# giuvecchio/PyPBR

Hardware: AMD Instinct MI355X
Metric: Mpixels/s Cook-Torrance eval, 4K maps (higher is better)
Workload: dtype f32

## Files before the change

### __graft_entry__.py

```python
import os
import subprocess
import sys

ROOT = os.path.dirname(os.path.abspath(__file__))
if ROOT not in sys.path:
    sys.path.insert(0, ROOT)


def build() -> None:
    subprocess.check_call(["make", "-s", "-j4", "-C", os.path.join(ROOT, "pypbr_amd", "csrc")])
    subprocess.check_call(["make", "-s", "-C", os.path.join(ROOT, "pypbr_amd", "csrc"), "torch_ops"])
    subprocess.check_call(["make", "-s", "-C", os.path.join(ROOT, "oracle")])
    boxcal_src, boxcal_so = os.path.join(ROOT, "tools", "boxcal.hip"), os.path.join(ROOT, "tools", "libboxcal.so")
    if not os.path.exists(boxcal_so) or os.path.getmtime(boxcal_so) < os.path.getmtime(boxcal_src):
        try:
            subprocess.check_call([os.environ.get("HIPCC", "/opt/rocm/bin/hipcc"), "-O3", "--offload-arch=gfx950", "-shared", "-fPIC", boxcal_src, "-o", boxcal_so])
        except (OSError, subprocess.CalledProcessError) as e:
            print("warning: tools/libboxcal.so (bench-side calibration helper, optional) did not build: %s" % e, file=sys.stderr)
    sys.path.insert(0, os.path.join(ROOT, "tools"))
    import check_isa
    report = check_isa.check()
    print("ISA check ok: %d hand-scheduled kernel instantiations; %s" % (sum(1 for r in report if "<" in r.split("vgpr")[0]), report[-1][:120]))
    import pypbr_amd
    from pypbr_amd import _native
    lib = _native.lib()
    for sym in _native.EXPORTS:
        getattr(lib, sym)
    assert lib.pbr_abi_version() == _native.ABI_VERSION
    from pypbr_amd import torch_ops
    assert torch_ops.available(), "pypbr_amd/_pbr_torch_ops.so did not build or load"
    import torch
    for op in ("cook_torrance", "cook_torrance_backward", "fold_gradient", "srgb_to_linear", "linear_to_srgb",
               "metallic_to_diffuse_specular", "diffuse_specular_to_basecolor_metallic", "colour_backward",
               "metallic_to_diffuse_specular_backward", "diffuse_specular_to_basecolor_metallic_backward", "resize", "resize_backward",
               "normal_from_height", "normal_from_height_backward", "normal_transform", "normal_transform_backward"):
        getattr(torch.ops.pbr_hip, op)
    print("build ok: %s (ABI %d), pypbr_amd %s" % (_native.LIB_PATH, lib.pbr_abi_version(), pypbr_amd.__version__))


def smoke() -> None:
    import torch
    sys.path.insert(0, os.path.join(ROOT, "oracle"))
    import torch_oracle
    from pypbr_amd.materials import BasecolorMetallicMaterial
    from pypbr_amd.models import CookTorranceBRDF

    assert torch.cuda.is_available(), "smoke() needs a ROCm device"
    g = torch.Generator().manual_seed(2024)
    H, W = 96, 128
    albedo = torch.rand(3, H, W, generator=g)
    nxy = torch.rand(2, H, W, generator=g) - 0.5
    normal = torch.cat([nxy, torch.ones(1, H, W)], 0)
    normal = normal / normal.norm(dim=0, keepdim=True)
    rough = torch.rand(1, H, W, generator=g) * 0.85 + 0.15
    metal = torch.rand(1, H, W, generator=g)
    view, light, inten = torch.tensor([0.0, 0.0, 1.0]), torch.tensor([0.1, 0.1, 1.0]), torch.tensor([1.0, 1.0, 1.0])

    mat = BasecolorMetallicMaterial(albedo=albedo, normal=normal, roughness=rough, metallic=metal).to("cuda:0")
    out = CookTorranceBRDF(light_type="point")(mat, view, light, inten, 1.0)
    torch.cuda.synchronize()
    assert out.shape == (3, H, W) and out.device.type == "cuda"
    ref = torch_oracle.cook_torrance(albedo, normal, rough, metal, None, view=view, light=light, intensity=inten,
                                     light_type="point", light_size=1.0)
# ... 10 lines not shown
```

### include/pbr_hip.h

```cpp
#ifndef PBR_HIP_H
#define PBR_HIP_H

#include <stddef.h>
#include <stdint.h>

#ifdef __cplusplus
extern "C" {
#endif

#define PBR_HIP_ABI_VERSION 9
#define PBR_MAX_LIGHTS 16

enum {
    PBR_OK = 0,
    PBR_ERR_NULL_MAP = -1,
    PBR_ERR_WORKFLOW = -2,
    PBR_ERR_LIGHT_TYPE = -3,
    PBR_ERR_SHAPE = -4,
    PBR_ERR_DTYPE = -5,
    PBR_ERR_CHANNELS = -6,
    PBR_ERR_NO_DEVICE = -7,
    PBR_ERR_UNSUPPORTED = -8
};

// ... 48 lines not shown
    int32_t n_lights;
    int32_t albedo_is_srgb;
    int32_t specular_is_srgb;
    int32_t return_srgb;

    pbr_map albedo;
    pbr_map normal;
    pbr_map roughness;
    pbr_map metallic;
    pbr_map specular;
    void *out;

    float view_dir[3];
    float light_size;
    float lights[PBR_MAX_LIGHTS][3];
    float intensities[PBR_MAX_LIGHTS][3];

    int32_t schedule;
    int32_t map_height;
    int32_t map_width;
    int32_t reserved;
    int64_t out_batch_stride;
    int64_t out_channel_stride;
    const void *device_params;
    const pbr_tuning *tuning;
} pbr_render_desc;

#define PBR_SCHEDULE_AUTO 0
#define PBR_SCHEDULE_LINEAR 1
#define PBR_SCHEDULE_XCD(c) (1 + (c))

int pbr_cook_torrance(const pbr_render_desc *desc, void *stream);

int pbr_cook_torrance_autotune(const pbr_render_desc *desc, void *stream, int32_t *schedule);

enum { PBR_BLEND_SIGN_COMPUTE = 0, PBR_BLEND_SIGN_GIVEN = 1 };
typedef struct pbr_blend_desc {
    pbr_map albedo, normal, roughness, metallic, specular;
    pbr_map mask;
    int32_t sign_mode;
    int32_t reserved;
} pbr_blend_desc;
int pbr_blend_normal_sign(const pbr_render_desc *desc, const pbr_blend_desc *blend, void *workspace, void *stream);
int pbr_cook_torrance_blend(const pbr_render_desc *desc, const pbr_blend_desc *blend, void *workspace, void *stream);

int pbr_blend_backward_serves(const pbr_render_desc *desc);
typedef struct pbr_map_grads { void *albedo, *normal, *roughness, *metallic, *specular; } pbr_map_grads;
int pbr_cook_torrance_blend_backward(const pbr_render_desc *desc, const pbr_blend_desc *blend, void *workspace, const void *grad_out,
                                     const pbr_map_grads *g_material1, const pbr_map_grads *g_material2, void *g_mask, void *stream);

int pbr_cook_torrance_backward(const pbr_render_desc *desc, const void *grad_out, void *g_albedo,
                               void *g_normal, void *g_roughness, void *g_metallic, void *g_specular,
                               void *stream);

size_t pbr_backward_folded_workspace_bytes(const pbr_render_desc *desc);
int pbr_cook_torrance_backward_folded(const pbr_render_desc *desc, const void *grad_out, void *g_albedo, void *g_normal,
                                      void *g_roughness, void *g_metallic, void *g_specular, void *workspace, void *stream);

size_t pbr_param_grad_workspace_bytes(const pbr_render_desc *desc);
int pbr_cook_torrance_backward_params(const pbr_render_desc *desc, const void *grad_out, void *g_albedo,
                                      void *g_normal, void *g_roughness, void *g_metallic, void *g_specular,
                                      void *g_params, void *workspace, void *stream);

size_t pbr_mse_step_workspace_bytes(const pbr_render_desc *desc);
int pbr_cook_torrance_mse_step(const pbr_render_desc *desc, const void *target, void *g_albedo, void *g_normal, void *g_roughness,
                               void *g_metallic, void *g_specular, void *loss, void *workspace, void *stream);
// ... 92 lines not shown
```

### pypbr_amd/_native.py

```python
import ctypes
import os

_HERE = os.path.dirname(os.path.abspath(__file__))
LIB_PATH = os.environ.get("PBR_HIP_LIB") or os.path.join(_HERE, "libpbr_hip.so")

ABI_VERSION = 9
RESIZE_TWO_PASS, RESIZE_STRIP, RESIZE_TWO_TAP, RESIZE_BAND_WALK, RESIZE_ROW_WALK = range(5)
MAX_LIGHTS = 16

F32, F16 = 0, 1
LIGHT_DIRECTIONAL, LIGHT_POINT = 0, 1
WORKFLOW_METALLIC, WORKFLOW_SPECULAR, WORKFLOW_CONVERTED = 0, 1, 2
(_TUNE_RESERVED_0, TUNE_BLOCK_LOG2, TUNE_F16_VEC, TUNE_LDS_BYTES, _TUNE_RESERVED_4, TUNE_BATCH_INNER, TUNE_SCALAR_BASE, TUNE_MAX_VEC, TUNE_BWD_RUN,
 TUNE_MSE_STREAM, TUNE_TILE_REPEAT, TUNE_RESIZE_UP2) = range(12)

TUNE_COUNT, TUNE_SLOTS, TUNE_UNSET = 12, 32, -2 ** 31
TUNE_NAMES = {"block_log2": TUNE_BLOCK_LOG2, "f16_vec": TUNE_F16_VEC, "lds_bytes": TUNE_LDS_BYTES, "batch_inner": TUNE_BATCH_INNER, "scalar_base": TUNE_SCALAR_BASE, "max_vec": TUNE_MAX_VEC,
              "bwd_run": TUNE_BWD_RUN, "mse_stream": TUNE_MSE_STREAM, "tile_repeat": TUNE_TILE_REPEAT, "resize_up2": TUNE_RESIZE_UP2}

OK = 0
ERR_NULL_MAP, ERR_WORKFLOW, ERR_LIGHT_TYPE, ERR_SHAPE, ERR_DTYPE, ERR_CHANNELS, ERR_NO_DEVICE = -1, -2, -3, -4, -5, -6, -7
ERR_UNSUPPORTED = -8

EXPORTS = (
    "pbr_cook_torrance", "pbr_srgb_to_linear", "pbr_linear_to_srgb", "pbr_metallic_to_specular",
    "pbr_specular_to_metallic", "pbr_decode_normal", "pbr_abi_version", "pbr_error_string",
    "pbr_kernel_name", "pbr_bytes_per_pixel", "pbr_set_tuning", "pbr_render_desc_size",
    "pbr_resize_workspace_bytes", "pbr_resize_bilinear", "pbr_resize_form", "pbr_cook_torrance_backward",
    "pbr_blend_maps", "pbr_blend_sigmoid_mask", "pbr_blend_gradient_mask", "pbr_cook_torrance_autotune",
    "pbr_cook_torrance_blend", "pbr_fold_gradient", "pbr_decode_normal_backward",
    "pbr_blend_normal_sign", "pbr_blend_backward_serves", "pbr_blend_maps_backward", "pbr_param_grad_workspace_bytes", "pbr_cook_torrance_backward_params",
    "pbr_srgb_to_linear_backward", "pbr_linear_to_srgb_backward", "pbr_metallic_to_specular_backward",
    "pbr_specular_to_metallic_backward", "pbr_resize_backward_workspace_bytes", "pbr_resize_bilinear_backward",
    "pbr_blend_sigmoid_mask_backward", "pbr_cook_torrance_blend_backward", "pbr_fold_gradient_typed",
    "pbr_mse_step_workspace_bytes", "pbr_cook_torrance_mse_step", "pbr_scale_by_device_scalar", "pbr_scale_list_by_device_scalar", "pbr_device_params_bytes", "pbr_prepare_device_params", "pbr_tuning_init", "pbr_build_id", "pbr_unpack_image",
    "pbr_backward_folded_workspace_bytes", "pbr_cook_torrance_backward_folded",
    "pbr_normal_from_height", "pbr_normal_from_height_backward", "pbr_normal_transform", "pbr_normal_transform_backward",
)


class PbrMap(ctypes.Structure):
    _fields_ = [("data", ctypes.c_void_p), ("batch_stride", ctypes.c_int64), ("channel_stride", ctypes.c_int64)]


class Tuning(ctypes.Structure):
    _fields_ = [("knob", ctypes.c_int32 * TUNE_SLOTS)]

    @classmethod
    def of(cls, **knobs):
        t = cls()
        for i in range(TUNE_SLOTS):
            t.knob[i] = TUNE_UNSET
        for name, value in knobs.items():
            t.knob[TUNE_NAMES[name]] = int(value)
        return t


class RenderDesc(ctypes.Structure):
    _fields_ = [
        ("abi_version", ctypes.c_int32), ("batch", ctypes.c_int32), ("height", ctypes.c_int32),
        ("width", ctypes.c_int32), ("height_total", ctypes.c_int32), ("y_offset", ctypes.c_int32),
        ("map_dtype", ctypes.c_int32), ("out_dtype", ctypes.c_int32), ("workflow", ctypes.c_int32),
        ("light_type", ctypes.c_int32), ("n_lights", ctypes.c_int32), ("albedo_is_srgb", ctypes.c_int32),
        ("specular_is_srgb", ctypes.c_int32), ("return_srgb", ctypes.c_int32),
        ("albedo", PbrMap), ("normal", PbrMap), ("roughness", PbrMap), ("metallic", PbrMap), ("specular", PbrMap),
        ("out", ctypes.c_void_p),
        ("view_dir", ctypes.c_float * 3), ("light_size", ctypes.c_float),
        ("lights", (ctypes.c_float * 3) * MAX_LIGHTS), ("intensities", (ctypes.c_float * 3) * MAX_LIGHTS),
        ("schedule", ctypes.c_int32), ("map_height", ctypes.c_int32), ("map_width", ctypes.c_int32),
        ("reserved", ctypes.c_int32),
# ... 16 lines not shown
BLEND_SIGN_COMPUTE, BLEND_SIGN_GIVEN = 0, 1


SCHEDULE_AUTO, SCHEDULE_LINEAR = 0, 1


def schedule_xcd(c: int) -> int:
    return 1 + c


class NativeLibraryError(RuntimeError):
    pass


_lib = None


def lib():
    global _lib
    if _lib is not None:
        return _lib
    import torch
    if not os.path.exists(LIB_PATH):
        raise NativeLibraryError(
            "%s is missing: build it with `python -c 'import __graft_entry__ as g; g.build()'` "
            "or `make -C pypbr_amd/csrc`.  pypbr_amd has no CPU fallback." % LIB_PATH)
    try:
        L = ctypes.CDLL(LIB_PATH)
    except OSError as e:
        raise NativeLibraryError("cannot load %s: %s" % (LIB_PATH, e)) from e
    vp, i32, i64, sz = ctypes.c_void_p, ctypes.c_int32, ctypes.c_int64, ctypes.c_size_t
    L.pbr_cook_torrance.argtypes = [ctypes.POINTER(RenderDesc), vp]
    L.pbr_cook_torrance.restype = ctypes.c_int
    L.pbr_cook_torrance_autotune.argtypes = [ctypes.POINTER(RenderDesc), vp, ctypes.POINTER(ctypes.c_int32)]
    L.pbr_cook_torrance_autotune.restype = ctypes.c_int
    L.pbr_cook_torrance_blend.argtypes = [ctypes.POINTER(RenderDesc), ctypes.POINTER(BlendDesc), vp, vp]
    L.pbr_cook_torrance_blend.restype = ctypes.c_int
    L.pbr_cook_torrance_blend_backward.argtypes = [ctypes.POINTER(RenderDesc), ctypes.POINTER(BlendDesc), vp, vp, ctypes.POINTER(MapGrads),
                                                   ctypes.POINTER(MapGrads), vp, vp]
    L.pbr_cook_torrance_blend_backward.restype = ctypes.c_int
    L.pbr_blend_normal_sign.argtypes = [ctypes.POINTER(RenderDesc), ctypes.POINTER(BlendDesc), vp, vp]
    L.pbr_blend_normal_sign.restype = ctypes.c_int
    L.pbr_blend_backward_serves.argtypes = [ctypes.POINTER(RenderDesc)]
    L.pbr_blend_backward_serves.restype = ctypes.c_int
    L.pbr_param_grad_workspace_bytes.argtypes = [ctypes.POINTER(RenderDesc)]
    L.pbr_param_grad_workspace_bytes.restype = ctypes.c_size_t
    L.pbr_cook_torrance_backward_params.argtypes = [ctypes.POINTER(RenderDesc), vp, vp, vp, vp, vp, vp, vp, vp, vp]
    L.pbr_cook_torrance_backward_params.restype = ctypes.c_int
    L.pbr_fold_gradient.argtypes = [vp, vp, i32, i32, i32, i32, i32, i32, ctypes.c_int, vp]
    L.pbr_fold_gradient.restype = ctypes.c_int
    L.pbr_mse_step_workspace_bytes.argtypes = [ctypes.POINTER(RenderDesc)]
    L.pbr_mse_step_workspace_bytes.restype = ctypes.c_size_t
    L.pbr_cook_torrance_mse_step.argtypes = [ctypes.POINTER(RenderDesc), vp, vp, vp, vp, vp, vp, vp, vp, vp]
    L.pbr_cook_torrance_mse_step.restype = ctypes.c_int
    L.pbr_scale_by_device_scalar.argtypes = [vp, sz, ctypes.c_int, vp, vp]
    L.pbr_scale_by_device_scalar.restype = ctypes.c_int
    L.pbr_scale_list_by_device_scalar.argtypes = [ctypes.POINTER(vp), ctypes.POINTER(sz), ctypes.c_int, ctypes.c_int, vp, vp]
    L.pbr_scale_list_by_device_scalar.restype = ctypes.c_int
    L.pbr_device_params_bytes.argtypes = []
    L.pbr_device_params_bytes.restype = ctypes.c_size_t
    L.pbr_prepare_device_params.argtypes = [ctypes.POINTER(RenderDesc), vp, vp, vp, i32, vp, vp]
    L.pbr_prepare_device_params.restype = ctypes.c_int
    L.pbr_fold_gradient_typed.argtypes = [vp, vp, i32, i32, i32, i32, i32, i32, ctypes.c_int, ctypes.c_int, vp]
    L.pbr_fold_gradient_typed.restype = ctypes.c_int
    L.pbr_cook_torrance_backward.argtypes = [ctypes.POINTER(RenderDesc), vp, vp, vp, vp, vp, vp, vp]
    L.pbr_cook_torrance_backward.restype = ctypes.c_int
# ... 128 lines not shown
```

### pypbr_amd/csrc/cook_torrance.hip

```cpp
#include <hip/hip_runtime.h>

#include <algorithm>

#include "ct_launch.hpp"

namespace pbr {

static constexpr int kKnobRules[PBR_TUNE_COUNT] = {
     1,  0,  8,  -1,  0,  -1,
     1,  8,  -1,  1,  -1,  1};
std::atomic<int> g_knobs[PBR_TUNE_COUNT] = {
    {kKnobRules[0]}, {kKnobRules[1]}, {kKnobRules[2]}, {kKnobRules[3]}, {kKnobRules[4]}, {kKnobRules[5]}, {kKnobRules[6]}, {kKnobRules[7]},
    {kKnobRules[8]}, {kKnobRules[9]}, {kKnobRules[10]}, {kKnobRules[11]}};
thread_local const pbr_tuning *t_tuning = nullptr;

struct KernelEntry { KernelFn fn; const char *name; };

template <int LIGHT, int WF, typename TI, typename TO>
static KernelFn pick_variant(int vec, bool multi) {
    if constexpr (sizeof(TI) == 2) {
        if (vec == 8 && !multi) {
            return cook_torrance_kernel<LIGHT, WF, TI, TO, 8, false, true>;
        }
    }
    if (vec == 1) return multi ? cook_torrance_kernel<LIGHT, WF, TI, TO, 1, true, false>
                               : cook_torrance_kernel<LIGHT, WF, TI, TO, 1, false, false>;
    return multi ? cook_torrance_kernel<LIGHT, WF, TI, TO, 4, true, true> : cook_torrance_kernel<LIGHT, WF, TI, TO, 4, false, true>;
}

template <int LIGHT, int WF>
static KernelFn pick_types(int in_dt, int out_dt, int vec, bool multi) {
    if (in_dt == PBR_F32) return out_dt == PBR_F32 ? pick_variant<LIGHT, WF, float, float>(vec, multi)
                                                   : pick_variant<LIGHT, WF, float, __half>(vec, multi);
    if (out_dt == PBR_F32) return pick_variant<LIGHT, WF, __half, float>(vec, multi);
    return pick_variant<LIGHT, WF, __half, __half>(vec, multi);
}

static KernelEntry pick_kernel(const pbr_render_desc *d, int vec) {
    static thread_local char name[96];
    static const char *const wf_names[3] = {"metallic", "specular", "converted"};
    const bool multi = d->n_lights > 1, point = d->light_type == PBR_LIGHT_POINT;
    const int idt = d->map_dtype, odt = d->out_dtype;
    const int nb = batch_group(d, vec);
    if (repeat_inner(d)) {
        std::snprintf(name, sizeof(name), "ctr_%s_%s_%s_%s_v4%s", point ? "point" : "directional", wf_names[d->workflow],
                      idt == PBR_F32 ? "f32" : "f16", odt == PBR_F32 ? "f32" : "f16", multi ? "_multi" : "");
        return KernelEntry{pick_repeat_kernel(d), name};
    }
    if (nb) {
        std::snprintf(name, sizeof(name), "ctb_%s_%s_%s_%s_v2_b%d", point ? "point" : "directional", wf_names[d->workflow],
                      idt == PBR_F32 ? "f32" : "f16", odt == PBR_F32 ? "f32" : "f16", nb);
        return KernelEntry{pick_batch_kernel(d, nb), name};
    }
    std::snprintf(name, sizeof(name), "ct_%s_%s_%s_%s_v%d%s", point ? "point" : "directional", wf_names[d->workflow],
                  idt == PBR_F32 ? "f32" : "f16", odt == PBR_F32 ? "f32" : "f16", vec, multi ? "_multi" : "");
    return KernelEntry{with_light_workflow(d, [&](auto L, auto W) -> KernelFn { return pick_types<L(), W()>(idt, odt, vec, multi); }), name};
}

}

namespace pbr {
struct HostParams { float view[3]; float lights[PBR_MAX_LIGHTS][3]; float inten[PBR_MAX_LIGHTS][3]; };
__global__ __launch_bounds__(64) void prepare_device_params_kernel(const float *__restrict__ view, const float *__restrict__ lights,
                                                                   const float *__restrict__ inten, int intensity_rows, int n_lights, int light_type,
                                                                   const HostParams hp, DevParams *__restrict__ out) {
    const int i = threadIdx.x;
    float raw[3];
    for (int c = 0; c < 3; ++c) raw[c] = view ? view[c] : hp.view[c];
    float V[3];
    normalize_host(raw, V);
    auto intensity = [&](int l, int c) { return inten ? inten[3 * (intensity_rows == 1 ? 0 : l) + c] : hp.inten[l][c]; };
    if (i == 0) {
        int grey = 1;
        for (int l = 0; l < n_lights; ++l)
            if (intensity(l, 0) != intensity(l, 1) || intensity(l, 0) != intensity(l, 2)) grey = 0;
        for (int c = 0; c < 3; ++c) { out->V[c] = V[c]; out->raw_view[c] = raw[c]; }
        out->grey = grey;
    }
    if (i < n_lights) {
        float L[3], I[3];
        for (int c = 0; c < 3; ++c) { L[c] = lights ? lights[3 * i + c] : hp.lights[i][c]; I[c] = intensity(i, c); }
        LightU u;
        fold_light(light_type, V, L, I, u);
        out->lights[i] = u;
        for (int c = 0; c < 3; ++c) out->raw_lights[i][c] = L[c];
    }
}
}

extern "C" {

int pbr_cook_torrance(const pbr_render_desc *d, void *stream) {
    using namespace pbr;
    const TuningScope tuning(d);
    const int rc = validate(d);
    if (rc != PBR_OK) return rc;
    if (nan_light_size(d)) return fill_result_nan(d, static_cast<hipStream_t>(stream));
    const int vec = pick_vec(d);
    KArgs k;
    if (repeat_inner(d)) {
        fill_repeat_args(d, k);
        if (k.n_tiles < 0) return PBR_ERR_SHAPE;
        const KernelEntry e = pick_kernel(d, 4);
        hipLaunchKernelGGL(e.fn, dim3((unsigned)k.n_tiles, 1, 1), dim3(1u << k.bt_log2, 1, 1), g_lds_bytes >= 0 ? (size_t)g_lds_bytes : 0,
                           static_cast<hipStream_t>(stream), k);
        return launch_status();
    }
    const int nb = batch_group(d, vec);
    if (nb) {
        pbr_render_desc g = *d;
        g.batch = d->batch / nb;
        fill_args(&g, 2, k);
        if (g_scalar_base != 2) k.sbase = 0;
    } else {
        fill_args(d, vec, k);
    }
    if (k.n_tiles < 0) return PBR_ERR_SHAPE;
    const bool tiled = k.tiled != 0;
    const KernelEntry e = pick_kernel(d, vec);
    const bool fp32_one_light = d->map_dtype == PBR_F32 && d->n_lights == 1 && k.bt_log2 == 6 && !tiled;
    size_t lds = g_lds_bytes >= 0 ? (size_t)g_lds_bytes : (fp32_one_light ? kLdsFor11WavesPerCu : 0);
    if (k.xpose) lds = std::max(lds, (size_t)kXposeLdsPerWave << (k.bt_log2 - 6));
    hipLaunchKernelGGL(e.fn, dim3((unsigned)k.n_tiles, 1, 1), dim3(1u << k.bt_log2, 1, 1), lds,
                       static_cast<hipStream_t>(stream), k);
    return launch_status();
}

int pbr_cook_torrance_autotune(const pbr_render_desc *d, void *stream, int32_t *schedule) {
    using namespace pbr;
    const int rc = validate(d);
    if (rc != PBR_OK) return rc;
    if (!schedule) return PBR_ERR_NULL_MAP;
    const int32_t cands[2] = {PBR_SCHEDULE_LINEAR, PBR_SCHEDULE_XCD(6)};
    float best[2] = {3.4e38f, 3.4e38f};
    hipStream_t st = static_cast<hipStream_t>(stream);
    hipEvent_t e0, e1;
    hipError_t created = hipEventCreate(&e0);
    if (created == hipSuccess) created = hipEventCreate(&e1);
    if (created != hipSuccess) return call_status(created);
    pbr_render_desc t = *d;
    int err = PBR_OK;
    const int reps = 4;
    for (int round = 0; round < 3 && err == PBR_OK; ++round) {
        for (int c = 0; c < 2 && err == PBR_OK; ++c) {
            t.schedule = cands[c];
            if ((err = pbr_cook_torrance(&t, stream)) != PBR_OK) break;
            hipError_t he = hipEventRecord(e0, st);
            for (int i = 0; i < reps && err == PBR_OK; ++i) err = pbr_cook_torrance(&t, stream);
            if (he == hipSuccess) he = hipEventRecord(e1, st);
            if (he == hipSuccess) he = hipEventSynchronize(e1);
            float ms = 0.0f;
            if (he == hipSuccess) he = hipEventElapsedTime(&ms, e0, e1);
            if (he != hipSuccess) { err = hip_code(he); break; }
            if (ms < best[c]) best[c] = ms;
        }
    }
    (void)hipEventDestroy(e0); (void)hipEventDestroy(e1);
    if (err != PBR_OK) return err;
    *schedule = best[1] < best[0] ? cands[1] : cands[0];
    return PBR_OK;
}

const char *pbr_kernel_name(const pbr_render_desc *d) {
    const pbr::TuningScope tuning(d);
    if (pbr::validate(d) != PBR_OK) return nullptr;
    return pbr::pick_kernel(d, pbr::pick_vec(d)).name;
}

int pbr_bytes_per_pixel(const pbr_render_desc *d) {
    if (pbr::validate(d) != PBR_OK) return 0;
    const int ein = d->map_dtype == PBR_F32 ? 4 : 2, eout = d->out_dtype == PBR_F32 ? 4 : 2;
    int ch = 3 + 1;
    if (d->normal.data) ch += 3;
    ch += d->workflow == PBR_WORKFLOW_SPECULAR ? 3 : 1;
    if (pbr::is_tiled(d)) {
        const int64_t reps = ((int64_t)d->height_total / d->map_height) * ((int64_t)d->width / d->map_width);
        return (int)((ch * ein + reps - 1) / reps) + 3 * eout;
    }
    return ch * ein + 3 * eout;
}

int pbr_set_tuning(int knob, int value) {
    if (knob < 0 || knob >= PBR_TUNE_COUNT) return -1;
    return pbr::g_knobs[knob].exchange(value == PBR_TUNE_UNSET ? pbr::kKnobRules[knob] : value, std::memory_order_relaxed);
}

void pbr_tuning_init(pbr_tuning *t) {
    if (!t) return;
    for (int i = 0; i < PBR_TUNE_SLOTS; ++i) t->knob[i] = PBR_TUNE_UNSET;
}

size_t pbr_device_params_bytes(void) { return sizeof(pbr::DevParams); }

int pbr_prepare_device_params(const pbr_render_desc *d, const void *view_dir, const void *lights, const void *intensities,
                              int32_t intensity_rows, void *block, void *stream) {
    using namespace pbr;
    if (!d || !block) return PBR_ERR_NULL_MAP;
    if (d->abi_version != PBR_HIP_ABI_VERSION || d->n_lights < 1 || d->n_lights > PBR_MAX_LIGHTS) return PBR_ERR_SHAPE;
    if (d->light_type != PBR_LIGHT_POINT && d->light_type != PBR_LIGHT_DIRECTIONAL) return PBR_ERR_LIGHT_TYPE;
    if (intensities && intensity_rows != 1 && intensity_rows != d->n_lights) return PBR_ERR_SHAPE;
    HostParams hp;
    for (int c = 0; c < 3; ++c) hp.view[c] = d->view_dir[c];
    for (int i = 0; i < PBR_MAX_LIGHTS; ++i)
        for (int c = 0; c < 3; ++c) { hp.lights[i][c] = d->lights[i][c]; hp.inten[i][c] = d->intensities[i][c]; }
    hipLaunchKernelGGL(prepare_device_params_kernel, dim3(1), dim3(64), 0, static_cast<hipStream_t>(stream), static_cast<const float *>(view_dir),
                       static_cast<const float *>(lights), static_cast<const float *>(intensities), (int)intensity_rows, (int)d->n_lights,
                       (int)d->light_type, hp, static_cast<DevParams *>(block));
    return launch_status();
}

}
```

### pypbr_amd/models.py

```python
import collections
import os
import threading
import weakref
from abc import ABC
from typing import Optional

import torch
import torch.nn as nn
from torch import Tensor

from . import _native
from . import functional as F_
from .materials import MaterialBase, _normalised


DEVICE_CACHE_CAP = int(os.environ.get("PBR_DEVICE_CACHE_CAP", str(4 << 30)))
_DEVICE_CACHES = collections.OrderedDict()


def _touch_device_cache(material):
    if id(material) in _DEVICE_CACHES:
        _DEVICE_CACHES.move_to_end(id(material))


def _register_device_cache(material, nbytes):
    _DEVICE_CACHES.pop(id(material), None)
    for key in [k for k, (ref, _) in _DEVICE_CACHES.items() if ref() is None or "_device_cache" not in ref().__dict__]:
        del _DEVICE_CACHES[key]
    _DEVICE_CACHES[id(material)] = (weakref.ref(material), nbytes)
    total = sum(n for _, n in _DEVICE_CACHES.values())
    while total > DEVICE_CACHE_CAP and len(_DEVICE_CACHES) > 1:
        _, (ref, n) = _DEVICE_CACHES.popitem(last=False)
        if ref() is not None:
            ref().__dict__.pop("_device_cache", None)
        total -= n


def _upload_together(tensors, compute):
    host = [i for i, t in enumerate(tensors) if t is not None and t.device.type == "cpu"]
    moved = [None if t is None else (t if t.device == compute or t.device.type == "cpu" else t.to(compute)) for t in tensors]
    if host:
        views, _ = F_.upload_packed([tensors[i] for i in host], compute)
        for i, v in zip(host, views):
            moved[i] = v
    return tuple(moved)

# ... 6 lines not shown

    def __init__(self, light_type: str = "point", override_device: torch.device = None):
        super().__init__()
        self.light_type = light_type.lower()
        if self.light_type not in ["directional", "point"]:
            raise ValueError(
                f"Unsupported light_type: {self.light_type}. Must be 'directional' or 'point'."
            )
        self.override_device = override_device

    @staticmethod
    def _staged(material, maps, blend, compute):
        tensors = tuple(maps) + tuple(blend or ())
        if any(t is not None and t.requires_grad for t in tensors):
            moved = tuple(None if t is None else t.to(compute) for t in tensors)
            return moved[:5], (None if blend is None else moved[5:])
        versions = tuple(None if t is None else F_.version_of(t) for t in tensors)
        wanted = (F_.CACHING["device_maps"] or material.__dict__.get("_cache_on_device", False))
        cacheable = wanted and all(v is not None for t, v in zip(tensors, versions) if t is not None)
        hit = material.__dict__.get("_device_cache") if cacheable else None
        if (hit is not None and hit[0] == compute and hit[1] == versions and len(hit[2]) == len(tensors)
                and all((r is None and t is None) or (r is not None and r() is t) for r, t in zip(hit[2], tensors))):
            moved = hit[3]
            _touch_device_cache(material)
        else:
            moved = _upload_together(tensors, compute)
            if cacheable:
                refs = tuple(None if t is None else weakref.ref(t) for t in tensors)
                material.__dict__["_device_cache"] = (compute, versions, refs, moved)
                _register_device_cache(material, sum(t.numel() * t.element_size() for t in moved if t is not None))
        return moved[:5], (None if blend is None else moved[5:])

    PLAN_REUSE = True

    @staticmethod
    def _host_values(v):
        if isinstance(v, torch.Tensor):
            if v.is_cuda or v.requires_grad:
                return None
            return v.tolist()
        if isinstance(v, (list, tuple)):
            return [list(r) if isinstance(r, (list, tuple)) else r for r in v]
        return None

    def _reuse_plan(self, material, view_dir, light, intensity, light_size, return_srgb):
        d = material.__dict__
        store = d.get("_store")
        if store is None or d.get("_lazy_blend") is not None or d.get("_raw_normal") or self.override_device is not None:
            return None
        vals = (self._host_values(view_dir), self._host_values(light), self._host_values(intensity))
        if vals[0] is None or vals[1] is None or vals[2] is None:
            return None
        albedo, normal, rough = store.get("albedo"), store.get("normal", False), store.get("roughness")
        second = store.get("metallic")
        if second is None:
            second = store.get("specular")
        if albedo is None or normal is False or rough is None or second is None or not albedo.is_cuda or albedo.device != material.device:
            return None
        maps = (albedo, normal, rough, second)
        grad = torch.is_grad_enabled()
        for t in maps:
            if t is not None and (t.device != albedo.device or t.dtype.itemsize > 4 or not t.is_floating_point() or (grad and t.requires_grad)
                                  or t.stride(-1) != 1 or t.stride(-2) != t.shape[-1]):
                return None
        key = (self.light_type, light_size, bool(return_srgb), bool(material.albedo_is_srgb), bool(getattr(material, "specular_is_srgb", True)),
               d.get("_lazy_tile", (1, 1)), "metallic" in store and store["metallic"] is not None,
# ... 5 lines not shown
        if hit is None:
            if d.get("_plan_seen") != key:
                d["_plan_seen"] = key
                return None
            return key
        if not hit[3].acquire(False):
            return None
        plan = hit[1]
        try:
            last = hit[2]
            if last != vals:
                if len(F_._host_vec3(vals[1], rows=-1)) != plan.desc.n_lights:
                    return key
                F_.refill_parameters(plan.desc, *vals)
                hit[2] = vals
            dev = plan.device
            out = torch.empty(hit[4], dtype=torch.float32, device=dev)
            plan.out = out
            plan.desc.out = out.data_ptr()
            if torch.cuda.current_device() == dev.index:
                plan.launch()
            else:
                with torch.cuda.device(dev):
                    plan.launch()
            return out[0] if plan._squeeze else out
        finally:
            plan.out = None
            hit[3].release()

    def forward(self, material, view_dir: Tensor, light_dir_or_position: Tensor, light_intensity: Tensor,
                light_size: Optional[float] = None, return_srgb: bool = True) -> Tensor:
        reuse_key = None
        if self.PLAN_REUSE and isinstance(material, MaterialBase):
            got = self._reuse_plan(material, view_dir, light_dir_or_position, light_intensity, light_size, return_srgb)
            if isinstance(got, torch.Tensor):
                return got
            reuse_key = got
        out_device = _normalised(self.override_device or material.device)

        pending = material.__dict__.get("_lazy_blend")
        blend = None
        if pending is not None:
            first, (second, mask) = material.__dict__["_store"], pending
            albedo, normal, roughness = first["albedo"], first["normal"], first["roughness"]
            metallic, specular = first.get("metallic"), None
            if metallic is None:
                specular = first["specular"]
            specular_is_srgb = bool(getattr(material, "specular_is_srgb", True))
            blend = (second["albedo"], second["normal"], second["roughness"], second.get("metallic") if metallic is not None else None,
                     second.get("specular") if metallic is None else None, mask)
        else:
            store = material.__dict__.get("_store") if isinstance(material, MaterialBase) else None
            if store is not None and material._has_pending():
                store = {**store, **material._resident(keep=False)}

            def probe(name):
                if store is None:
                    return getattr(material, name)
                if name not in store:
                    raise AttributeError(f"'{type(material).__name__}' object has no attribute '{name}'")
                return store[name]

            def has(name):
                return (name in store) if store is not None else hasattr(material, name)

            roughness = probe("roughness")
# ... 2 lines not shown
            specular_is_srgb = True
            if has("metallic") and probe("metallic") is not None:
                metallic = probe("metallic")
            elif has("specular") and probe("specular") is not None:
                specular = probe("specular")
                specular_is_srgb = bool(getattr(material, "specular_is_srgb", True))
            else:
                raise ValueError("Material must have either 'metallic' or 'specular' property.")
            albedo = store.get("albedo") if store is not None else material._maps.get("albedo")
            if albedo is None:
                raise AttributeError(f"'{type(material).__name__}' material has no albedo map")

        if out_device.type == "cuda":
            compute = out_device
        else:
            _native.require_device()
            compute = torch.device("cuda", torch.cuda.current_device())

        maps = (albedo, normal, roughness, metallic, specular)
        if any(t is not None and t.device != compute for t in maps + (blend or ())):
            maps, blend = self._staged(material, maps, blend, compute)
        if reuse_key is not None and blend is None and albedo.numel() > 0:
            plan = F_.plan_cook_torrance(*maps, view_dir=view_dir, light=light_dir_or_position, light_intensity=light_intensity,
                                         light_type=self.light_type, light_size=light_size, albedo_is_srgb=bool(material.albedo_is_srgb),
                                         specular_is_srgb=specular_is_srgb, return_srgb=return_srgb, tile=getattr(material, "lazy_tile", (1, 1)))
            with torch.cuda.device(plan.device):
                color = plan.launch()
            four = (maps[0], maps[1], maps[2], maps[3] if maps[3] is not None else maps[4])
            held = tuple(t for t in four if t is not None)
            if plan._param_block is None and all(p is None or any(p.data_ptr() == t.data_ptr() for t in held) for p in plan._keep):
                plan._keep = ()
                material.__dict__["_plan_cache"] = [reuse_key, plan, (self._host_values(view_dir), self._host_values(light_dir_or_position),
                                                                     self._host_values(light_intensity)), threading.Lock(), tuple(plan.out.shape),
                                                    tuple(None if t is None else weakref.ref(t) for t in four)]
            plan.out = None
            return color
        color = F_.cook_torrance(
            *maps,
            view_dir=view_dir, light=light_dir_or_position, light_intensity=light_intensity,
            light_type=self.light_type, light_size=light_size,
            albedo_is_srgb=bool(material.albedo_is_srgb), specular_is_srgb=specular_is_srgb,
            return_srgb=return_srgb, tile=getattr(material, "lazy_tile", (1, 1)),
            blend=blend)
        if color.device == out_device:
            return color
        return F_.to_host(color, out_device) if out_device.type == "cpu" else color.to(out_device)
```

Baseline: 147,300.

## Add native C-extension fast path for repeated Cook-Torrance plan reuse calls

```diff
diff --git a/__graft_entry__.py b/__graft_entry__.py
--- a/__graft_entry__.py
+++ b/__graft_entry__.py
@@ -10,6 +10,7 @@
 def build() -> None:
     subprocess.check_call(["make", "-s", "-j4", "-C", os.path.join(ROOT, "pypbr_amd", "csrc")])
     subprocess.check_call(["make", "-s", "-C", os.path.join(ROOT, "pypbr_amd", "csrc"), "torch_ops"])
+    subprocess.check_call(["make", "-s", "-C", os.path.join(ROOT, "pypbr_amd", "csrc"), "fast_call"])
     subprocess.check_call(["make", "-s", "-C", os.path.join(ROOT, "oracle")])
     boxcal_src, boxcal_so = os.path.join(ROOT, "tools", "boxcal.hip"), os.path.join(ROOT, "tools", "libboxcal.so")
     if not os.path.exists(boxcal_so) or os.path.getmtime(boxcal_so) < os.path.getmtime(boxcal_src):
@@ -29,6 +30,8 @@
     assert lib.pbr_abi_version() == _native.ABI_VERSION
     from pypbr_amd import torch_ops
     assert torch_ops.available(), "pypbr_amd/_pbr_torch_ops.so did not build or load"
+    from pypbr_amd import models
+    assert models._fast is not None and models._fast.abi_version() == _native.ABI_VERSION, "pypbr_amd/_pbr_fast_call.so did not build or load"
     import torch
     for op in ("cook_torrance", "cook_torrance_backward", "fold_gradient", "srgb_to_linear", "linear_to_srgb",
                "metallic_to_diffuse_specular", "diffuse_specular_to_basecolor_metallic", "colour_backward",
diff --git a/include/pbr_hip.h b/include/pbr_hip.h
--- a/include/pbr_hip.h
+++ b/include/pbr_hip.h
@@ -104,6 +104,12 @@
 
 int pbr_cook_torrance(const pbr_render_desc *desc, void *stream);
 
+typedef struct pbr_prepared pbr_prepared;
+int pbr_cook_torrance_prepare(const pbr_render_desc *desc, pbr_prepared **handle);
+int pbr_prepared_launch(pbr_prepared *handle, void *out, void *stream);
+int pbr_prepared_set_parameters(pbr_prepared *handle, const float *view_dir, const float *lights, const float *intensities, int32_t n_lights);
+void pbr_prepared_free(pbr_prepared *handle);
+
 int pbr_cook_torrance_autotune(const pbr_render_desc *desc, void *stream, int32_t *schedule);
 
 enum { PBR_BLEND_SIGN_COMPUTE = 0, PBR_BLEND_SIGN_GIVEN = 1 };
diff --git a/pypbr_amd/_native.py b/pypbr_amd/_native.py
--- a/pypbr_amd/_native.py
+++ b/pypbr_amd/_native.py
@@ -36,6 +36,7 @@
     "pbr_mse_step_workspace_bytes", "pbr_cook_torrance_mse_step", "pbr_scale_by_device_scalar", "pbr_scale_list_by_device_scalar", "pbr_device_params_bytes", "pbr_prepare_device_params", "pbr_tuning_init", "pbr_build_id", "pbr_unpack_image",
     "pbr_backward_folded_workspace_bytes", "pbr_cook_torrance_backward_folded",
     "pbr_normal_from_height", "pbr_normal_from_height_backward", "pbr_normal_transform", "pbr_normal_transform_backward",
+    "pbr_cook_torrance_prepare", "pbr_prepared_launch", "pbr_prepared_set_parameters", "pbr_prepared_free",
 )
 
 
@@ -118,6 +119,14 @@
     vp, i32, i64, sz = ctypes.c_void_p, ctypes.c_int32, ctypes.c_int64, ctypes.c_size_t
     L.pbr_cook_torrance.argtypes = [ctypes.POINTER(RenderDesc), vp]
     L.pbr_cook_torrance.restype = ctypes.c_int
+    L.pbr_cook_torrance_prepare.argtypes = [ctypes.POINTER(RenderDesc), ctypes.POINTER(vp)]
+    L.pbr_cook_torrance_prepare.restype = ctypes.c_int
+    L.pbr_prepared_launch.argtypes = [vp, vp, vp]
+    L.pbr_prepared_launch.restype = ctypes.c_int
+    L.pbr_prepared_set_parameters.argtypes = [vp, ctypes.POINTER(ctypes.c_float), ctypes.POINTER(ctypes.c_float), ctypes.POINTER(ctypes.c_float), i32]
+    L.pbr_prepared_set_parameters.restype = ctypes.c_int
+    L.pbr_prepared_free.argtypes = [vp]
+    L.pbr_prepared_free.restype = None
     L.pbr_cook_torrance_autotune.argtypes = [ctypes.POINTER(RenderDesc), vp, ctypes.POINTER(ctypes.c_int32)]
     L.pbr_cook_torrance_autotune.restype = ctypes.c_int
     L.pbr_cook_torrance_blend.argtypes = [ctypes.POINTER(RenderDesc), ctypes.POINTER(BlendDesc), vp, vp]
diff --git a/pypbr_amd/csrc/cook_torrance.hip b/pypbr_amd/csrc/cook_torrance.hip
--- a/pypbr_amd/csrc/cook_torrance.hip
+++ b/pypbr_amd/csrc/cook_torrance.hip
@@ -1,6 +1,7 @@
 #include <hip/hip_runtime.h>
 
 #include <algorithm>
+#include <new>
 
 #include "ct_launch.hpp"
 
@@ -57,7 +58,74 @@
     return KernelEntry{with_light_workflow(d, [&](auto L, auto W) -> KernelFn { return pick_types<L(), W()>(idt, odt, vec, multi); }), name};
 }
 
-}
+struct Launch {
+    KernelFn fn;
+    unsigned grid, block;
+    size_t lds;
+    bool nan_fill;
+    KArgs k;
+};
+
+static int prepare_launch(const pbr_render_desc *d, Launch &l) {
+    const int rc = validate(d);
+    if (rc != PBR_OK) return rc;
+    l.nan_fill = nan_light_size(d);
+    if (l.nan_fill) return PBR_OK;
+    const int vec = pick_vec(d);
+    KArgs &k = l.k;
+    if (repeat_inner(d)) {
+        fill_repeat_args(d, k);
+        if (k.n_tiles < 0) return PBR_ERR_SHAPE;
+        l.fn = pick_kernel(d, 4).fn;
+        l.grid = (unsigned)k.n_tiles; l.block = 1u << k.bt_log2;
+        l.lds = g_lds_bytes >= 0 ? (size_t)g_lds_bytes : 0;
+        return PBR_OK;
+    }
+    const int nb = batch_group(d, vec);
+    if (nb) {
+        pbr_render_desc g = *d;
+        g.batch = d->batch / nb;
+        fill_args(&g, 2, k);
+        if (g_scalar_base != 2) k.sbase = 0;
+    } else {
+        fill_args(d, vec, k);
+    }
+    if (k.n_tiles < 0) return PBR_ERR_SHAPE;
+    const bool tiled = k.tiled != 0;
+    l.fn = pick_kernel(d, vec).fn;
+    const bool fp32_one_light = d->map_dtype == PBR_F32 && d->n_lights == 1 && k.bt_log2 == 6 && !tiled;
+    size_t lds = g_lds_bytes >= 0 ? (size_t)g_lds_bytes : (fp32_one_light ? kLdsFor11WavesPerCu : 0);
+    if (k.xpose) lds = std::max(lds, (size_t)kXposeLdsPerWave << (k.bt_log2 - 6));
+    l.grid = (unsigned)k.n_tiles; l.block = 1u << k.bt_log2; l.lds = lds;
+    return PBR_OK;
+}
+
+static int enqueue(const Launch &l, const pbr_render_desc *d, hipStream_t stream) {
+    if (l.nan_fill) return fill_result_nan(d, stream);
+    hipLaunchKernelGGL(l.fn, dim3(l.grid, 1, 1), dim3(l.block, 1, 1), l.lds, stream, l.k);
+    return launch_status();
+}
+
+static std::atomic<unsigned> g_knob_generation{0};
+
+}
+
+struct pbr_prepared {
+    pbr_render_desc desc;
+    pbr_tuning tuning;
+    bool has_tuning;
+    bool out_aligned;
+    unsigned knob_generation;
+    pbr::Launch launch;
+
+    int resolve() {
+        desc.tuning = has_tuning ? &tuning : nullptr;
+        const pbr::TuningScope scope(&desc);
+        knob_generation = pbr::g_knob_generation.load(std::memory_order_relaxed);
+        out_aligned = pbr::is_aligned(desc.out, 16);
+        return pbr::prepare_launch(&desc, launch);
+    }
+};
 
 namespace pbr {
 struct HostParams { float view[3]; float lights[PBR_MAX_LIGHTS][3]; float inten[PBR_MAX_LIGHTS][3]; };
@@ -93,38 +161,52 @@
 int pbr_cook_torrance(const pbr_render_desc *d, void *stream) {
     using namespace pbr;
     const TuningScope tuning(d);
+    Launch l;
+    const int rc = prepare_launch(d, l);
+    if (rc != PBR_OK) return rc;
+    return enqueue(l, d, static_cast<hipStream_t>(stream));
+}
+
+int pbr_cook_torrance_prepare(const pbr_render_desc *d, pbr_prepared **handle) {
+    using namespace pbr;
+    if (!handle) return PBR_ERR_NULL_MAP;
+    *handle = nullptr;
     const int rc = validate(d);
     if (rc != PBR_OK) return rc;
-    if (nan_light_size(d)) return fill_result_nan(d, static_cast<hipStream_t>(stream));
-    const int vec = pick_vec(d);
-    KArgs k;
-    if (repeat_inner(d)) {
-        fill_repeat_args(d, k);
-        if (k.n_tiles < 0) return PBR_ERR_SHAPE;
-        const KernelEntry e = pick_kernel(d, 4);
-        hipLaunchKernelGGL(e.fn, dim3((unsigned)k.n_tiles, 1, 1), dim3(1u << k.bt_log2, 1, 1), g_lds_bytes >= 0 ? (size_t)g_lds_bytes : 0,
-                           static_cast<hipStream_t>(stream), k);
-        return launch_status();
-    }
-    const int nb = batch_group(d, vec);
-    if (nb) {
-        pbr_render_desc g = *d;
-        g.batch = d->batch / nb;
-        fill_args(&g, 2, k);
-        if (g_scalar_base != 2) k.sbase = 0;
-    } else {
-        fill_args(d, vec, k);
-    }
-    if (k.n_tiles < 0) return PBR_ERR_SHAPE;
-    const bool tiled = k.tiled != 0;
-    const KernelEntry e = pick_kernel(d, vec);
-    const bool fp32_one_light = d->map_dtype == PBR_F32 && d->n_lights == 1 && k.bt_log2 == 6 && !tiled;
-    size_t lds = g_lds_bytes >= 0 ? (size_t)g_lds_bytes : (fp32_one_light ? kLdsFor11WavesPerCu : 0);
-    if (k.xpose) lds = std::max(lds, (size_t)kXposeLdsPerWave << (k.bt_log2 - 6));
-    hipLaunchKernelGGL(e.fn, dim3((unsigned)k.n_tiles, 1, 1), dim3(1u << k.bt_log2, 1, 1), lds,
-                       static_cast<hipStream_t>(stream), k);
-    return launch_status();
-}
+    if (is_tiled(d) || d->device_params) return PBR_ERR_UNSUPPORTED;
+    pbr_prepared *h = new (std::nothrow) pbr_prepared;
+    if (!h) return hip_code(hipErrorOutOfMemory);
+    h->desc = *d;
+    h->has_tuning = d->tuning != nullptr;
+    if (h->has_tuning) h->tuning = *d->tuning;
+    const int ready = h->resolve();
+    if (ready != PBR_OK) { delete h; return ready; }
+    *handle = h;
+    return PBR_OK;
+}
+
+int pbr_prepared_launch(pbr_prepared *h, void *out, void *stream) {
+    using namespace pbr;
+    if (!h || !out) return PBR_ERR_NULL_MAP;
+    h->desc.out = out;
+    if (h->knob_generation != g_knob_generation.load(std::memory_order_relaxed) || is_aligned(out, 16) != h->out_aligned) {
+        const int rc = h->resolve();
+        if (rc != PBR_OK) return rc;
+    }
+    h->launch.k.out = out;
+    return enqueue(h->launch, &h->desc, static_cast<hipStream_t>(stream));
+}
+
+int pbr_prepared_set_parameters(pbr_prepared *h, const float *view_dir, const float *lights, const float *intensities, int32_t n_lights) {
+    if (!h || !view_dir || !lights || !intensities) return PBR_ERR_NULL_MAP;
+    if (n_lights != h->desc.n_lights) return PBR_ERR_SHAPE;
+    for (int c = 0; c < 3; ++c) h->desc.view_dir[c] = view_dir[c];
+    for (int i = 0; i < n_lights; ++i)
+        for (int c = 0; c < 3; ++c) { h->desc.lights[i][c] = lights[3 * i + c]; h->desc.intensities[i][c] = intensities[3 * i + c]; }
+    return h->resolve();
+}
+
+void pbr_prepared_free(pbr_prepared *h) { delete h; }
 
 int pbr_cook_torrance_autotune(const pbr_render_desc *d, void *stream, int32_t *schedule) {
     using namespace pbr;
@@ -182,7 +264,9 @@
 
 int pbr_set_tuning(int knob, int value) {
     if (knob < 0 || knob >= PBR_TUNE_COUNT) return -1;
-    return pbr::g_knobs[knob].exchange(value == PBR_TUNE_UNSET ? pbr::kKnobRules[knob] : value, std::memory_order_relaxed);
+    const int previous = pbr::g_knobs[knob].exchange(value == PBR_TUNE_UNSET ? pbr::kKnobRules[knob] : value, std::memory_order_relaxed);
+    pbr::g_knob_generation.fetch_add(1, std::memory_order_release);
+    return previous;
 }
 
 void pbr_tuning_init(pbr_tuning *t) {
diff --git a/pypbr_amd/csrc/fast_call.cpp b/pypbr_amd/csrc/fast_call.cpp
--- /dev/null
+++ b/pypbr_amd/csrc/fast_call.cpp
@@ -0,0 +1,238 @@
+#include <Python.h>
+
+#include <ATen/ATen.h>
+#include <ATen/hip/EmptyTensor.h>
+#include <c10/core/GradMode.h>
+#include <c10/hip/HIPFunctions.h>
+#include <c10/hip/HIPGuard.h>
+#include <c10/hip/HIPStream.h>
+#include <torch/csrc/Device.h>
+#include <torch/csrc/autograd/python_variable.h>
+
+#include <atomic>
+#include <cstring>
+#include <vector>
+
+#include "../../include/pbr_hip.h"
+
+namespace {
+
+constexpr const char *kCapsule = "pypbr_amd.fast_plan";
+
+struct MapSeen {
+    PyObject *object = nullptr;
+    PyObject *weak = nullptr;
+    const void *data = nullptr;
+    std::vector<int64_t> sizes, strides;
+    at::ScalarType dtype = at::kFloat;
+};
+
+struct FastPlan {
+    pbr_prepared *handle = nullptr;
+    MapSeen maps[4];
+    c10::Device device{c10::kCUDA, 0};
+    PyObject *light_type = nullptr, *light_size = nullptr, *one_tile = nullptr;
+    bool return_srgb = true, albedo_srgb = true, specular_srgb = true, has_metallic = true;
+    std::vector<int64_t> out_shape;
+    int n_lights = 1;
+    bool have_last = false;
+    float last[3 + 6 * PBR_MAX_LIGHTS];
+    std::atomic_flag busy = ATOMIC_FLAG_INIT;
+
+    ~FastPlan() {
+        pbr_prepared_free(handle);
+        for (MapSeen &m : maps) Py_XDECREF(m.weak);
+        Py_XDECREF(light_type); Py_XDECREF(light_size); Py_XDECREF(one_tile);
+    }
+};
+
+struct Names { PyObject *store, *lazy_blend, *raw_normal, *lazy_tile, *plan_cache, *albedo, *normal, *roughness, *metallic, *specular,
+                        *albedo_is_srgb, *specular_is_srgb, *device, *light_type, *override_device; } S;
+
+void destroy_plan(PyObject *capsule) { delete static_cast<FastPlan *>(PyCapsule_GetPointer(capsule, kCapsule)); }
+
+inline PyObject *dict_get(PyObject *d, PyObject *name) { return PyDict_GetItemWithError(d, name); }
+
+int flag_of(PyObject *material, PyObject *mdict, PyObject *name, int missing) {
+    PyObject *v = dict_get(mdict, name);
+    if (v) return PyObject_IsTrue(v);
+    if (PyErr_Occurred()) return -1;
+    v = PyObject_GetAttr(material, name);
+    if (!v) {
+        if (missing < 0 || !PyErr_ExceptionMatches(PyExc_AttributeError)) return -1;
+        PyErr_Clear();
+        return missing;
+    }
+    const int r = PyObject_IsTrue(v);
+    Py_DECREF(v);
+    return r;
+}
+
+bool same_value(PyObject *a, PyObject *b) {
+    if (a == b) return true;
+    const int r = PyObject_RichCompareBool(a, b, Py_EQ);
+    if (r < 0) PyErr_Clear();
+    return r == 1;
+}
+
+const float *host_floats(PyObject *o, int64_t &numel) {
+    if (!THPVariable_Check(o)) return nullptr;
+    const at::Tensor &t = THPVariable_Unpack(o);
+    if (!t.defined() || !t.device().is_cpu() || t.requires_grad() || t.scalar_type() != at::kFloat || !t.is_contiguous() || t.layout() != at::kStrided)
+        return nullptr;
+    numel = t.numel();
+    return static_cast<const float *>(t.data_ptr());
+}
+
+bool weak_is(PyObject *weak, PyObject *object) { return weak && PyWeakref_GetObject(weak) == object; }
+
+PyObject *build(PyObject *, PyObject *const *args, Py_ssize_t nargs) {
+    if (nargs != 10) { PyErr_SetString(PyExc_TypeError, "build() takes 10 arguments"); return nullptr; }
+    const auto *desc = static_cast<const pbr_render_desc *>(PyLong_AsVoidPtr(args[0]));
+    if (!desc) { if (!PyErr_Occurred()) PyErr_SetString(PyExc_ValueError, "null descriptor"); return nullptr; }
+    PyObject *maps = args[1], *shape = args[2];
+    if (!PyTuple_Check(maps) || PyTuple_GET_SIZE(maps) != 4 || !PyTuple_Check(shape) || !THPDevice_Check(args[3])) {
+        PyErr_SetString(PyExc_TypeError, "build(): maps is a tuple of 4, out_shape a tuple, material_device a torch.device");
+        return nullptr;
+    }
+    auto plan = std::make_unique<FastPlan>();
+    for (Py_ssize_t i = 0; i < PyTuple_GET_SIZE(shape); ++i) {
+        plan->out_shape.push_back(PyLong_AsLongLong(PyTuple_GET_ITEM(shape, i)));
+        if (PyErr_Occurred()) return nullptr;
+    }
+    bool first = true;
+    for (int i = 0; i < 4; ++i) {
+        PyObject *o = PyTuple_GET_ITEM(maps, i);
+        if (o == Py_None) continue;
+        if (!THPVariable_Check(o)) { PyErr_SetString(PyExc_TypeError, "build(): maps must be tensors or None"); return nullptr; }
+        const at::Tensor &t = THPVariable_Unpack(o);
+        if (!t.is_cuda()) Py_RETURN_NONE;
+        MapSeen &m = plan->maps[i];
+        m.object = o;
+        if (!(m.weak = PyWeakref_NewRef(o, nullptr))) return nullptr;
+        m.data = t.data_ptr(); m.sizes = t.sizes().vec(); m.strides = t.strides().vec(); m.dtype = t.scalar_type();
+        if (first) { plan->device = t.device(); first = false; }
+        else if (t.device() != plan->device) Py_RETURN_NONE;
+    }
+    if (first || reinterpret_cast<THPDevice *>(args[3])->device != plan->device || !plan->device.has_index()) Py_RETURN_NONE;
+    plan->light_type = Py_NewRef(args[4]);
+    plan->light_size = Py_NewRef(args[5]);
+    if (!(plan->one_tile = Py_BuildValue("(ii)", 1, 1))) return nullptr;
+    const int flags[4] = {PyObject_IsTrue(args[6]), PyObject_IsTrue(args[7]), PyObject_IsTrue(args[8]), PyObject_IsTrue(args[9])};
+    for (int f : flags) if (f < 0) return nullptr;
+    plan->return_srgb = flags[0]; plan->albedo_srgb = flags[1]; plan->specular_srgb = flags[2]; plan->has_metallic = flags[3];
+    plan->n_lights = desc->n_lights;
+    if (desc->out_dtype != PBR_F32) Py_RETURN_NONE;
+    const int rc = pbr_cook_torrance_prepare(desc, &plan->handle);
+    if (rc == PBR_ERR_UNSUPPORTED) Py_RETURN_NONE;
+    if (rc != PBR_OK) { PyErr_Format(PyExc_RuntimeError, "pbr_cook_torrance_prepare: %s (%d)", pbr_error_string(rc), rc); return nullptr; }
+    PyObject *capsule = PyCapsule_New(plan.get(), kCapsule, destroy_plan);
+    if (capsule) plan.release();
+    return capsule;
+}
+
+PyObject *call(PyObject *, PyObject *const *args, Py_ssize_t nargs) {
+    if (nargs != 8) { PyErr_SetString(PyExc_TypeError, "call() takes 8 arguments"); return nullptr; }
+    PyObject *brdf = args[0], *material = args[1], *mdict = args[2];
+    if (!PyDict_Check(mdict)) Py_RETURN_NONE;
+    PyObject *entry = dict_get(mdict, S.plan_cache);
+    if (!entry || !PyList_Check(entry) || PyList_GET_SIZE(entry) < 7) { if (PyErr_Occurred()) return nullptr; Py_RETURN_NONE; }
+    PyObject *capsule = PyList_GET_ITEM(entry, 6);
+    if (!PyCapsule_CheckExact(capsule)) Py_RETURN_NONE;
+    auto *plan = static_cast<FastPlan *>(PyCapsule_GetPointer(capsule, kCapsule));
+    if (!plan) return nullptr;
+
+    PyObject *store = dict_get(mdict, S.store), *v;
+    if (!store || !PyDict_Check(store)) { if (PyErr_Occurred()) return nullptr; Py_RETURN_NONE; }
+    if ((v = dict_get(mdict, S.lazy_blend)) && v != Py_None) Py_RETURN_NONE;
+    if ((v = dict_get(mdict, S.raw_normal))) { const int r = PyObject_IsTrue(v); if (r < 0) return nullptr; if (r) Py_RETURN_NONE; }
+    if ((v = dict_get(mdict, S.lazy_tile)) && !same_value(v, plan->one_tile)) Py_RETURN_NONE;
+    if (PyErr_Occurred()) return nullptr;
+    if (!(v = PyObject_GetAttr(brdf, S.override_device))) return nullptr;
+    Py_DECREF(v);
+    if (v != Py_None) Py_RETURN_NONE;
+    if (!(v = PyObject_GetAttr(brdf, S.light_type))) return nullptr;
+    const bool same_light_type = same_value(v, plan->light_type);
+    Py_DECREF(v);
+    if (!same_light_type || !same_value(args[6], plan->light_size)) Py_RETURN_NONE;
+    const int rs = PyObject_IsTrue(args[7]), as = flag_of(material, mdict, S.albedo_is_srgb, -1), ss = flag_of(material, mdict, S.specular_is_srgb, 1);
+    if (rs < 0 || as < 0 || ss < 0) return nullptr;
+    if ((rs != 0) != plan->return_srgb || (as != 0) != plan->albedo_srgb || (ss != 0) != plan->specular_srgb) Py_RETURN_NONE;
+
+    PyObject *now[4] = {dict_get(store, S.albedo), dict_get(store, S.normal), dict_get(store, S.roughness), dict_get(store, S.metallic)};
+    if (!now[1]) Py_RETURN_NONE;
+    const bool has_metallic = now[3] && now[3] != Py_None;
+    if (!has_metallic) now[3] = dict_get(store, S.specular);
+    if (PyErr_Occurred()) return nullptr;
+    if (has_metallic != plan->has_metallic) Py_RETURN_NONE;
+    const bool grad = c10::GradMode::is_enabled();
+    for (int i = 0; i < 4; ++i) {
+        const MapSeen &m = plan->maps[i];
+        PyObject *o = now[i] == Py_None ? nullptr : now[i];
+        if (i != 1 && !o) Py_RETURN_NONE;
+        if (o != m.object) Py_RETURN_NONE;
+        if (!o) continue;
+        if (!weak_is(m.weak, o) || !THPVariable_Check(o)) Py_RETURN_NONE;
+        const at::Tensor &t = THPVariable_Unpack(o);
+        if (!t.defined() || t.device() != plan->device || t.scalar_type() != m.dtype || t.data_ptr() != m.data || t.sizes() != at::IntArrayRef(m.sizes) ||
+            t.strides() != at::IntArrayRef(m.strides) || (grad && t.requires_grad()))
+            Py_RETURN_NONE;
+    }
+    v = dict_get(mdict, S.device);
+    if (!v || !THPDevice_Check(v) || reinterpret_cast<THPDevice *>(v)->device != plan->device) { if (PyErr_Occurred()) return nullptr; Py_RETURN_NONE; }
+
+    int64_t nv = 0, nl = 0, ni = 0;
+    const float *view = host_floats(args[3], nv), *lights = host_floats(args[4], nl), *inten = host_floats(args[5], ni);
+    const int L = plan->n_lights;
+    if (!view || !lights || !inten || nv != 3 || nl != 3 * L || (ni != 3 * L && ni != 3)) Py_RETURN_NONE;
+    float vals[3 + 6 * PBR_MAX_LIGHTS];
+    std::memcpy(vals, view, 3 * sizeof(float));
+    std::memcpy(vals + 3, lights, 3 * L * sizeof(float));
+    for (int i = 0; i < L; ++i) std::memcpy(vals + 3 + 3 * L + 3 * i, inten + (ni == 3 ? 0 : 3 * i), 3 * sizeof(float));
+
+    if (plan->busy.test_and_set(std::memory_order_acquire)) Py_RETURN_NONE;
+    struct Release { std::atomic_flag &f; ~Release() { f.clear(std::memory_order_release); } } release{plan->busy};
+    try {
+        const size_t bytes = (3 + 6 * (size_t)L) * sizeof(float);
+        if (!plan->have_last || std::memcmp(plan->last, vals, bytes) != 0) {
+            const int rc = pbr_prepared_set_parameters(plan->handle, vals, vals + 3, vals + 3 + 3 * L, L);
+            if (rc != PBR_OK) { PyErr_Format(PyExc_RuntimeError, "pbr_prepared_set_parameters: %s (%d)", pbr_error_string(rc), rc); return nullptr; }
+            std::memcpy(plan->last, vals, bytes);
+            plan->have_last = true;
+        }
+        const c10::DeviceIndex index = plan->device.index();
+        c10::hip::OptionalHIPGuard guard;
+        if (c10::hip::current_device() != index) guard.set_index(index);
+        at::Tensor out = at::Tensor(at::detail::empty_cuda(plan->out_shape, at::kFloat, plan->device, std::nullopt));
+        const int rc = pbr_prepared_launch(plan->handle, out.data_ptr(), c10::hip::getCurrentHIPStream(index).stream());
+        if (rc != PBR_OK) { PyErr_Format(PyExc_RuntimeError, "pbr_prepared_launch: %s (%d)", pbr_error_string(rc), rc); return nullptr; }
+        return THPVariable_Wrap(std::move(out));
+    } catch (const std::exception &e) {
+        PyErr_SetString(PyExc_RuntimeError, e.what());
+        return nullptr;
+    }
+}
+
+PyObject *abi_version(PyObject *, PyObject *) { return PyLong_FromLong(pbr_abi_version()); }
+
+PyMethodDef kMethods[] = {
+    {"build", reinterpret_cast<PyCFunction>(reinterpret_cast<void (*)()>(build)), METH_FASTCALL,
+     "build(desc_address, maps, out_shape, material_device, light_type, light_size, return_srgb, albedo_is_srgb, specular_is_srgb, has_metallic) -> state | None"},
+    {"call", reinterpret_cast<PyCFunction>(reinterpret_cast<void (*)()>(call)), METH_FASTCALL,
+     "call(brdf, material, material.__dict__, view_dir, light, light_intensity, light_size, return_srgb) -> Tensor | None (not mine)"},
+    {"abi_version", abi_version, METH_NOARGS, "pbr_abi_version() of the library this module is linked against"},
+    {nullptr, nullptr, 0, nullptr}};
+
+PyModuleDef kModule = {PyModuleDef_HEAD_INIT, "_pbr_fast_call", "Native hit path of CookTorranceBRDF's plan reuse.", -1, kMethods};
+
+}
+
+PyMODINIT_FUNC PyInit__pbr_fast_call(void) {
+    PyObject **slots[] = {&S.store, &S.lazy_blend, &S.raw_normal, &S.lazy_tile, &S.plan_cache, &S.albedo, &S.normal, &S.roughness, &S.metallic,
+                          &S.specular, &S.albedo_is_srgb, &S.specular_is_srgb, &S.device, &S.light_type, &S.override_device};
+    const char *names[] = {"_store", "_lazy_blend", "_raw_normal", "_lazy_tile", "_plan_cache", "albedo", "normal", "roughness", "metallic",
+                           "specular", "albedo_is_srgb", "specular_is_srgb", "device", "light_type", "override_device"};
+    for (size_t i = 0; i < sizeof(names) / sizeof(names[0]); ++i)
+        if (!(*slots[i] = PyUnicode_InternFromString(names[i]))) return nullptr;
+    return PyModule_Create(&kModule);
+}
diff --git a/pypbr_amd/models.py b/pypbr_amd/models.py
--- a/pypbr_amd/models.py
+++ b/pypbr_amd/models.py
@@ -1,4 +1,5 @@
 import collections
+import ctypes
 import os
 import threading
 import weakref
@@ -12,6 +13,13 @@
 from . import _native
 from . import functional as F_
 from .materials import MaterialBase, _normalised
+
+try:
+    from . import _pbr_fast_call as _fast
+    if _fast.abi_version() != _native.ABI_VERSION:
+        _fast = None
+except ImportError:
+    _fast = None
 
 
 DEVICE_CACHE_CAP = int(os.environ.get("PBR_DEVICE_CACHE_CAP", str(4 << 30)))
@@ -84,6 +92,7 @@
         return moved[:5], (None if blend is None else moved[5:])
 
     PLAN_REUSE = True
+    NATIVE_CALL = True
 
     @staticmethod
     def _host_values(v):
@@ -155,6 +164,10 @@
                 light_size: Optional[float] = None, return_srgb: bool = True) -> Tensor:
         reuse_key = None
         if self.PLAN_REUSE and isinstance(material, MaterialBase):
+            if self.NATIVE_CALL and _fast is not None:
+                got = _fast.call(self, material, material.__dict__, view_dir, light_dir_or_position, light_intensity, light_size, return_srgb)
+                if got is not None:
+                    return got
             got = self._reuse_plan(material, view_dir, light_dir_or_position, light_intensity, light_size, return_srgb)
             if isinstance(got, torch.Tensor):
                 return got
@@ -223,7 +236,12 @@
                 plan._keep = ()
                 material.__dict__["_plan_cache"] = [reuse_key, plan, (self._host_values(view_dir), self._host_values(light_dir_or_position),
                                                                      self._host_values(light_intensity)), threading.Lock(), tuple(plan.out.shape),
-                                                    tuple(None if t is None else weakref.ref(t) for t in four)]
+                                                    tuple(None if t is None else weakref.ref(t) for t in four), None]
+                if _fast is not None:
+                    shape = tuple(plan.out.shape[1:]) if plan._squeeze else tuple(plan.out.shape)
+                    material.__dict__["_plan_cache"][6] = _fast.build(
+                        ctypes.addressof(plan.desc), four, shape, material.device, self.light_type, light_size, bool(return_srgb),
+                        bool(material.albedo_is_srgb), bool(getattr(material, "specular_is_srgb", True)), maps[3] is not None)
             plan.out = None
             return color
         color = F_.cook_torrance(
```

Measured after the change: 147,100. No clear change (-0.1%).
